# XuZhang1211/PVPUFormer

Hardware: AMD Instinct MI355X
Metric: 448x448 images/sec fwd+bwd, ViT-B VPUFormer (higher is better)
Workload: dtype bf16

## Files before the change

include/vpu_hip.h:

```cpp
#ifndef VPU_HIP_H
#define VPU_HIP_H
#include <stdint.h>

#ifdef __cplusplus
extern "C" {
#endif

#define VPU_BF16 0
#define VPU_F32 1

#define VPU_EPI_BIAS 1
#define VPU_EPI_PREACT 2
#define VPU_EPI_GELU 4
#define VPU_EPI_RELU 8
#define VPU_EPI_DGELU 16
#define VPU_EPI_DRELU 32
#define VPU_EPI_RESID 64
#define VPU_EPI_AFFINE 128
#define VPU_EPI_ACCUM 256
#define VPU_EPI_OUT_F32 512
#define VPU_EPI_SAVE_DGELU 1024
#define VPU_EPI_MULAUX 2048

typedef struct vpu_gemm_desc {
// ... 162 lines not shown
                             void* stream);
int vpu_pixel_shuffle2_gn_stats(const void* in, void* out, const float* bias, double* stats, int32_t B, int32_t h, int32_t w,
                                int32_t C, int32_t dtype, void* stream);
int vpu_groupnorm_apply(const void* x, const float* w, const float* b, void* y, float* mean, float* rstd, const double* stats,
                        int32_t B, int64_t HW, int32_t C, float eps, int32_t gelu, int32_t dtype, void* stream);
int vpu_pixel_unshuffle2_nblk(int32_t C);
int vpu_pixel_unshuffle2_sums(const void* in, void* out, float* part, int32_t B, int32_t h, int32_t w, int32_t C,
                              int32_t dtype, void* stream);
int vpu_groupnorm_nchunk(void);
int vpu_groupnorm_fwd(const void* x, const float* w, const float* b, void* y, float* mean, float* rstd, double* stats,
                      int32_t B, int64_t HW, int32_t C, float eps, int32_t gelu, int32_t dtype, void* stream);
int vpu_groupnorm_bwd(const void* dy, const void* x, const float* w, const float* b, const float* mean,
                      const float* rstd, void* dx, float* part, double* stats, int32_t B, int64_t HW, int32_t C,
                      int32_t gelu, int32_t dtype, void* stream);
int vpu_bilinear_cl_fwd(const void* in, int32_t ld_in, void* out, int32_t ld_out, int32_t B, int32_t h, int32_t w,
                        int32_t H, int32_t W, int32_t C, int32_t dtype, void* stream);
int vpu_bilinear_cl_bwd(const void* dout, int32_t ld_out, void* din, int32_t ld_in, int32_t B, int32_t h, int32_t w,
                        int32_t H, int32_t W, int32_t C, int32_t dtype, void* stream);
int vpu_upsum_relu(void* io, const void* const* z, const int32_t* h, const int32_t* w, int32_t n, int32_t B, int32_t H,
                   int32_t W, int32_t C, int32_t dtype, void* stream);
int vpu_head_grad_fused(const void* dfn, const void* y, const float* inv, const float* dout, const void* x, const float* w,
                        const float* mask, void* dx, float* part, float* part_b, int64_t rows, int64_t HW, int32_t C,
                        int32_t dtype, void* stream);
int vpu_gate_stats(const void* Q, const void* Kt, float* cg, int32_t* argq, float* sg, int32_t* argc, int32_t B,
                   int32_t nq, int32_t N, int32_t C, int32_t dtype, void* stream);
int vpu_gate_apply(const void* x, const float* cg, const float* sg, void* out, int32_t B, int32_t N, int32_t C,
                   int32_t dtype, void* stream);
int vpu_gate_bwd(const void* dout, const void* x, const float* cg, const int32_t* argq, const float* sg,
                 const int32_t* argc, void* dx, int32_t accum, void* dQ, void* dK, float* part, int32_t B, int32_t nq,
                 int32_t N, int32_t C, int32_t dtype, void* stream);
int vpu_gate_fwd_n(const void* const* Q, const void* const* K, const void* x, void* const* out, float* cg, int32_t* argq,
                   float* sg, int32_t* argc, int32_t n, int32_t B, int32_t nq, int32_t N, int32_t C, int32_t dtype, void* stream);
int vpu_gate_bwd_n(const void* const* dout, const void* x, const float* cg, const int32_t* argq, const float* sg,
                   const int32_t* argc, void* dx, int32_t accum, void* const* dQ, void* const* dK, float* part, int32_t n,
                   int32_t B, int32_t nq, int32_t N, int32_t C, int32_t dtype, void* stream);
int vpu_convseg_fwd(const void* x, const float* w, const float* bias, const float* mask, float* out, int64_t rows,
                    int64_t HW, int32_t C, int32_t dtype, void* stream);
int vpu_convseg_bwd_nblk(int64_t rows);
int vpu_convseg_bwd(const float* dout, const void* x, const float* w, const float* mask, void* dx, int32_t accum,
                    float* part, float* part_b, int64_t rows, int64_t HW, int32_t C, int32_t dtype, void* stream);

int vpu_upsample_ac_fwd(const float* in, float* out, int64_t planes, int32_t h, int32_t w, int32_t H, int32_t W,
                        void* stream);
int vpu_upsample_ac_bwd(const float* dout, float* din, int64_t planes, int32_t h, int32_t w, int32_t H, int32_t W,
                        void* stream);
int vpu_p2cl_fwd_bwd(const float* prob, const float* gt, const int32_t* slot_mask_idx, const float* override_masks,
// ... 28 lines not shown
```

pvpuformer_amd/_lib.py:

```python
import ctypes as C
import os

_HERE = os.path.dirname(os.path.abspath(__file__))
LIB_PATH = os.path.join(_HERE, os.environ.get("VPU_LIB_FILE") or
                        ("libvpu_hip_diag.so" if os.environ.get("VPU_LIB_DIAG", "0") == "1" else "libvpu_hip.so"))

BF16, F32 = 0, 1

EPI_BIAS, EPI_PREACT, EPI_GELU, EPI_RELU, EPI_DGELU, EPI_DRELU = 1, 2, 4, 8, 16, 32
EPI_RESID, EPI_AFFINE, EPI_ACCUM, EPI_OUT_F32 = 64, 128, 256, 512
EPI_SAVE_DGELU, EPI_MULAUX = 1024, 2048


class GemmDesc(C.Structure):
    _fields_ = [
        ("A", C.c_void_p), ("B", C.c_void_p), ("C", C.c_void_p), ("bias", C.c_void_p), ("resid", C.c_void_p),
        ("aux", C.c_void_p), ("preact", C.c_void_p),
        ("M", C.c_int32), ("N", C.c_int32), ("K", C.c_int32),
        ("lda", C.c_int32), ("ldb", C.c_int32), ("ldc", C.c_int32), ("ldr", C.c_int32), ("ldaux", C.c_int32),
        ("batch", C.c_int32), ("inner", C.c_int32),
        ("sAo", C.c_int64), ("sAi", C.c_int64), ("sBo", C.c_int64), ("sBi", C.c_int64),
        ("sCo", C.c_int64), ("sCi", C.c_int64), ("sRo", C.c_int64), ("sRi", C.c_int64),
        ("transA", C.c_int32), ("transB", C.c_int32), ("dtype", C.c_int32), ("flags", C.c_int32),
        ("resid_period", C.c_int32),
# ... 67 lines not shown
    "vpu_mask_bbox": [_P, _F, _P, _I, _P, _I, _I, _I, _P],
    "vpu_masked_argmax": [_P, _P, _P, _I, _I, _I, _P],
    "vpu_error_masks": [_P, _P, _P, _P, _I, _I, _P],
    "vpu_roi_resize_batched": [_P, _I, _P, _I, _I, _I, _I, _P],
    "vpu_roi_paste_batched": [_P, _I, _P, _I, _I, _F, _F, _I, _P],
    "vpu_click_keys_batched": [_P, _I, _P, _P, _P, _I, _I, _I, _P],
    "vpu_disk_maps": [_P, _P, _P, _I, _I, _I, _I, _F, _P],
    "vpu_patch_im2col": [_P, _P, _P, _I, _I, _I, _I, _I, _I, _P],
    "vpu_patch_im2col_prenorm": [_P, _P, _P, _I, _I, _I, _I, _I, _I, _P],
    "vpu_patch_im2col_floor": [_P, _P, _P, _I, _I, _I, _I, _I, _I, _I, _P],
    "vpu_window_permute": [_P, _P, _I, _I, _I, _I, _I, _I, _P],
    "vpu_space_to_depth2_crop": [_P, _P, _I, _I, _I, _I, _I, _P],
    "vpu_pixel_shuffle2": [_P, _P, _P, _I, _I, _I, _I, _I, _I, _P],
    "vpu_pixel_shuffle2_gn_stats": [_P, _P, _P, _P, _I, _I, _I, _I, _I, _P],
    "vpu_groupnorm_apply": [_P, _P, _P, _P, _P, _P, _P, _I, _L, _I, _F, _I, _I, _P],
    "vpu_pixel_unshuffle2_nblk": [_I],
    "vpu_pixel_unshuffle2_sums": [_P, _P, _P, _I, _I, _I, _I, _I, _P],
    "vpu_groupnorm_nchunk": [],
    "vpu_groupnorm_fwd": [_P, _P, _P, _P, _P, _P, _P, _I, _L, _I, _F, _I, _I, _P],
    "vpu_groupnorm_bwd": [_P, _P, _P, _P, _P, _P, _P, _P, _P, _I, _L, _I, _I, _I, _P],
    "vpu_bilinear_cl_fwd": [_P, _I, _P, _I, _I, _I, _I, _I, _I, _I, _I, _P],
    "vpu_bilinear_cl_bwd": [_P, _I, _P, _I, _I, _I, _I, _I, _I, _I, _I, _P],
    "vpu_head_grad_fused": [_P, _P, _P, _P, _P, _P, _P, _P, _P, _P, _L, _L, _I, _I, _P],
    "vpu_upsum_relu": [_P, C.POINTER(C.c_void_p), C.POINTER(C.c_int32), C.POINTER(C.c_int32), _I, _I, _I, _I, _I, _I, _P],
    "vpu_gate_stats": [_P, _P, _P, _P, _P, _P, _I, _I, _I, _I, _I, _P],
    "vpu_gate_apply": [_P, _P, _P, _P, _I, _I, _I, _I, _P],
    "vpu_gate_bwd": [_P, _P, _P, _P, _P, _P, _P, _I, _P, _P, _P, _I, _I, _I, _I, _I, _P],
    "vpu_gate_fwd_n": [C.POINTER(C.c_void_p), C.POINTER(C.c_void_p), _P, C.POINTER(C.c_void_p), _P, _P, _P, _P, _I, _I, _I, _I, _I, _I, _P],
    "vpu_gate_bwd_n": [C.POINTER(C.c_void_p), _P, _P, _P, _P, _P, _P, _I, C.POINTER(C.c_void_p), C.POINTER(C.c_void_p), _P, _I, _I, _I,
                       _I, _I, _I, _P],
    "vpu_convseg_fwd": [_P, _P, _P, _P, _P, _L, _L, _I, _I, _P],
    "vpu_convseg_bwd_nblk": [_L],
    "vpu_convseg_bwd": [_P, _P, _P, _P, _P, _I, _P, _P, _L, _L, _I, _I, _P],
    "vpu_upsample_ac_fwd": [_P, _P, _L, _I, _I, _I, _I, _P],
    "vpu_upsample_ac_bwd": [_P, _P, _L, _I, _I, _I, _I, _P],
    "vpu_p2cl_fwd_bwd": [_P, _P, _P, _P, _P, _P, _F, _I, _I, _I, _I, _P],
    "vpu_p2cl_up_nband": [_I, _I],
    "vpu_p2cl_up_fwd_bwd": [_P, _P, _P, _P, _P, _P, _F, _I, _I, _I, _I, _I, _I, _P],
    "vpu_nfl_dice_scratch_doubles": [_I],
    "vpu_nfl_dice_fwd_bwd": [_P, _P, _P, _P, _P, _F, _F, _I, _L, _P],
    "vpu_loss_finalize": [_P, _P, _I, _I, C.c_double, _F, _F, _F, _F, _P, _P],
    "vpu_adam_step": [_P, _P, _P, _P, _P, _L, _F, _F, _F, _F, _F, _I, _F, _P],
    "vpu_adam_step_groups": [_P, _P, _P, _P, _P, _L, _P, _P, _P, _I, _F, _F, _F, _I, _I, _F, _P],
    "vpu_adam_step_hyper": [_P, _P, _P, _P, _P, _L, _P, _P, _P, _P, _I, _F, _F, _F, _F, _I, _P],
    "vpu_gemm_set_option": [C.c_char_p, _I],
    "vpu_gemm_get_option": [C.c_char_p, C.POINTER(C.c_int32)],
# ... 40 lines not shown
```

pvpuformer_amd/csrc/spatial.hip:

```cpp
#include <stdlib.h>
#include "vpu_common.h"
#include "interp_ac.h"
#include "../../include/vpu_hip.h"

#define DISPATCH_T(dtype, ...)                                   \
    if ((dtype) == VPU_BF16) { using T = bf16_t; __VA_ARGS__ }   \
    else if ((dtype) == VPU_F32) { using T = float; __VA_ARGS__ } \
    else { vpu_set_error("bad dtype"); return VPU_ERR_ARG; }
#define ST reinterpret_cast<hipStream_t>(stream)

namespace {

__constant__ float c_mean[3] = {0.485f, 0.456f, 0.406f};
__constant__ float c_std[3] = {0.229f, 0.224f, 0.225f};

template <typename T, bool NORM = true, bool VEC = true>
__global__ __launch_bounds__(256) void patch_im2col_kernel(const float* __restrict__ img4,
                                                           const float* __restrict__ disks, T* __restrict__ cols,
                                                           int B, int H, int W, int P, int wg) {
    const int gw = W / P, gh = H / P;
    const int K3 = 3 * P * P, K3P = (K3 + 7) / 8 * 8;
    const int Tn = gw * gh, KK = 2 * K3P, chunks = KK / 8;
    const int64_t total = (int64_t)B * Tn * chunks;
    const int nwx = gw / wg;
// ... 711 lines not shown
            for (int u = 0; u < 2 * R; ++u) {
                const int X = Xs + u;
                if (X >= 0 && X < W) {
                    float g[8];
                    load8(rowp + (int64_t)X * ld_out, g);
                    const float ww = wy * wx[u];
#pragma unroll
                    for (int j = 0; j < 8; ++j) acc[j] += ww * g[j];
                }
            }
        }
    }
#pragma unroll
    for (int j = 0; j < 8; ++j) acc[j] += __shfl_xor(acc[j], 32, 64);
    if ((wave & 1) && lane < 32) {
#pragma unroll
        for (int j = 0; j < 8; ++j) red[wave >> 1][ck][j] = acc[j];
    }
    __syncthreads();
    if (!(wave & 1) && lane < 32 && live) {
#pragma unroll
        for (int j = 0; j < 8; ++j) acc[j] += red[wave >> 1][ck][j];
        store8(din + pix * ld_in + ck * 8, acc);
    }
}

template <typename T>
__global__ __launch_bounds__(256) void gate_colmax_kernel(const T* __restrict__ Q, float* __restrict__ cg,
                                                          int* __restrict__ argq, int B, int nq, int C) {
    const int64_t i = (int64_t)blockIdx.x * 256 + threadIdx.x;
    if (i >= (int64_t)B * C) return;
    const int c = (int)(i % C), b = (int)(i / C);
    float mx = -INFINITY;
    int am = 0;
#pragma unroll 8
    for (int q = 0; q < nq; ++q) {
        const float v = to_f32(Q[((int64_t)b * nq + q) * C + c]);
        if (v > mx) { mx = v; am = q; }
    }
    cg[i] = sigmoid_f(mx);
    argq[i] = am;
}
template <typename T>
__global__ __launch_bounds__(256) void gate_rowmax_kernel(const T* __restrict__ K, float* __restrict__ sg,
                                                          int* __restrict__ argc, int64_t rows, int C) {
    const int lane = threadIdx.x & 63;
// ... 539 lines not shown
            for (int j = 0; j < 8; ++j) {
                dwa[j] += d * xv[j] * mk[j];
                const float t = iv * (g[j] - yv[j] * sdot) + d * wv[j] * mk[j];
                o[j] = xv[j] > 0.f ? t : 0.f;
            }
            store8(dx + row * C + c8, o);
        }
    }
#pragma unroll
    for (int j = 0; j < 8; ++j)
        for (int o = lpr; o < 64; o <<= 1) dwa[j] += __shfl_xor(dwa[j], o, 64);
    dba = wave_sum(dba);
    if (sub == 0) {
#pragma unroll
        for (int j = 0; j < 8; ++j) red[wave][c8 + j] = dwa[j];
    }
    if (lane == 0) redb[wave] = dba;
    __syncthreads();
    for (int c = threadIdx.x; c < C; c += 256)
        part[(int64_t)blockIdx.x * C + c] = red[0][c] + red[1][c] + red[2][c] + red[3][c];
    if (threadIdx.x == 0) part_b[blockIdx.x] = redb[0] + redb[1] + redb[2] + redb[3];
}

__global__ __launch_bounds__(256) void upsample_ac_fwd_kernel(const float* __restrict__ in, float* __restrict__ out,
                                                              int64_t planes, int h, int w, int H, int W) {
    const float sh = ac_scale(h, H), sw = ac_scale(w, W);
    const int64_t total = planes * H * W;
    for (int64_t i = (int64_t)blockIdx.x * 256 + threadIdx.x; i < total; i += (int64_t)gridDim.x * 256) {
        const int X = (int)(i % W), Y = (int)((i / W) % H);
        const int64_t pl = i / ((int64_t)W * H);
        out[i] = ac_sample(in + pl * h * w, w, h, w, sh, sw, Y, X);
    }
}
__global__ __launch_bounds__(256) void upsample_ac_bwd_kernel(const float* __restrict__ dout, float* __restrict__ din,
                                                              int64_t planes, int h, int w, int H, int W) {
    const float sh = H > 1 ? (float)(h - 1) / (float)(H - 1) : 0.f;
    const float sw = W > 1 ? (float)(w - 1) / (float)(W - 1) : 0.f;
    const float fh = sh > 0.f ? 1.f / sh : 0.f, fw = sw > 0.f ? 1.f / sw : 0.f;
    const int64_t total = planes * h * w;
    const bool small = total < ((int64_t)1 << 31);
    for (int64_t i = (int64_t)blockIdx.x * 256 + threadIdx.x; i < total; i += (int64_t)gridDim.x * 256) {
        int x, y;
        int64_t pl;
        if (small) {
            const unsigned iu = (unsigned)i, q = iu / (unsigned)w;
            x = (int)(iu - q * (unsigned)w); y = (int)(q % (unsigned)h); pl = q / (unsigned)h;
// ... 221 lines not shown
    if ((R == 4 || R == 8) && R >= split_min && C == 256) {
        const unsigned g2 = (unsigned)(8 * ((((int64_t)B * h * w + 1) / 2 + 7) / 8));
        DISPATCH_T(dtype,
                   if (R == 4) bilinear_cl_bwd_int4_kernel<T, 4><<<g2, 256, 0, ST>>>((const T*)dout, ld_out, (T*)din, ld_in, B, h, w);
                   else bilinear_cl_bwd_int4_kernel<T, 8><<<g2, 256, 0, ST>>>((const T*)dout, ld_out, (T*)din, ld_in, B, h, w);)
        return vpu_check_launch("vpu_bilinear_cl_bwd");
    }
    if (R == 2 || R == 4 || R == 8) {
        const int64_t nb8 = 8 * (((total + 255) / 256 + 7) / 8);
        const unsigned gi = (unsigned)(nb8 < 16384 ? nb8 : 16384);
        DISPATCH_T(dtype,
                   if (R == 2) bilinear_cl_bwd_int_kernel<T, 2><<<gi, 256, 0, ST>>>(
                       (const T*)dout, ld_out, (T*)din, ld_in, B, h, w, C);
                   else if (R == 4) bilinear_cl_bwd_int_kernel<T, 4><<<gi, 256, 0, ST>>>(
                       (const T*)dout, ld_out, (T*)din, ld_in, B, h, w, C);
                   else bilinear_cl_bwd_int_kernel<T, 8><<<gi, 256, 0, ST>>>(
                       (const T*)dout, ld_out, (T*)din, ld_in, B, h, w, C);)
        return vpu_check_launch("vpu_bilinear_cl_bwd");
    }
    DISPATCH_T(dtype, bilinear_cl_bwd_kernel<T><<<vpu_grid_for(total, 256, 16384), 256, 0, ST>>>(
        (const T*)dout, ld_out, (T*)din, ld_in, B, h, w, H, W, C);)
    return vpu_check_launch("vpu_bilinear_cl_bwd");
}
extern "C" int vpu_gate_stats(const void* Q, const void* Kt, float* cg, int32_t* argq, float* sg, int32_t* argc,
                              int32_t B, int32_t nq, int32_t N, int32_t C, int32_t dtype, void* stream) {
    vpu_clear_stale_error();
    DISPATCH_T(dtype,
               gate_colmax_kernel<T><<<vpu_grid_for((int64_t)B * C, 256), 256, 0, ST>>>((const T*)Q, cg, argq, B, nq, C);
               gate_rowmax_kernel<T><<<(unsigned)(((int64_t)B * N + 3) / 4), 256, 0, ST>>>((const T*)Kt, sg, argc,
                                                                                          (int64_t)B * N, C);)
    return vpu_check_launch("vpu_gate_stats");
}
extern "C" int vpu_gate_apply(const void* x, const float* cg, const float* sg, void* out, int32_t B, int32_t N,
                              int32_t C, int32_t dtype, void* stream) {
    vpu_clear_stale_error();
    if (C % 8) { vpu_set_error("gate_apply: C % 8"); return VPU_ERR_ARG; }
    const int64_t total = (int64_t)B * N * (C / 8);
    DISPATCH_T(dtype, gate_apply_kernel<T><<<vpu_grid_for(total, 256, 16384), 256, 0, ST>>>((const T*)x, cg, sg, (T*)out,
                                                                                           B, N, C);)
    return vpu_check_launch("vpu_gate_apply");
}
extern "C" int vpu_gate_bwd(const void* dout, const void* x, const float* cg, const int32_t* argq, const float* sg,
                            const int32_t* argc, void* dx, int32_t accum, void* dQ, void* dK, float* part, int32_t B,
                            int32_t nq, int32_t N, int32_t C, int32_t dtype, void* stream) {
    vpu_clear_stale_error();
    if (C % 8 || C > 2048) { vpu_set_error("gate_bwd: C % 8, C <= 2048"); return VPU_ERR_ARG; }
// ... 84 lines not shown
        return vpu_check_launch("vpu_convseg_bwd");
    }
    DISPATCH_T(dtype, convseg_bwd_kernel<T><<<nblk, 256, 0, ST>>>(dout, (const T*)x, w, mask, (T*)dx, accum, part,
                                                                 part_b, rows, HW, C, nblk);)
    return vpu_check_launch("vpu_convseg_bwd");
}
extern "C" int vpu_head_grad_fused(const void* dfn, const void* y, const float* inv, const float* dout, const void* x,
                                   const float* w, const float* mask, void* dx, float* part, float* part_b, int64_t rows,
                                   int64_t HW, int32_t C, int32_t dtype, void* stream) {
    vpu_clear_stale_error();
    if (dtype != VPU_BF16 || !(C == 64 || C == 128 || C == 256 || C == 512) || !dfn || !y || !inv || !dout || !x || !w ||
        !dx || !part || !part_b || rows < 1 ||
        (reinterpret_cast<uintptr_t>(dfn) | reinterpret_cast<uintptr_t>(y) | reinterpret_cast<uintptr_t>(x) |
         reinterpret_cast<uintptr_t>(dx)) % 16 != 0 ||
        (reinterpret_cast<uintptr_t>(w) | reinterpret_cast<uintptr_t>(mask)) % 32 != 0) {
        vpu_set_error("head_grad_fused: bf16, C in {64,128,256,512}, 16-byte aligned maps, 32-byte aligned w / mask");
        return VPU_ERR_ARG;
    }
    const int nblk = vpu_convseg_bwd_nblk(rows);
    head_grad_fused_kernel<<<nblk, 256, 0, ST>>>((const bf16_t*)dfn, (const bf16_t*)y, inv, dout, (const bf16_t*)x, w, mask,
                                                 (bf16_t*)dx, part, part_b, rows, HW, C, nblk);
    return vpu_check_launch("vpu_head_grad_fused");
}
extern "C" int vpu_upsample_ac_fwd(const float* in, float* out, int64_t planes, int32_t h, int32_t w, int32_t H,
                                   int32_t W, void* stream) {
    vpu_clear_stale_error();
    upsample_ac_fwd_kernel<<<vpu_grid_for(planes * H * W, 256, 65536), 256, 0, ST>>>(in, out, planes, h, w, H, W);
    return vpu_check_launch("vpu_upsample_ac_fwd");
}
extern "C" int vpu_upsample_ac_bwd(const float* dout, float* din, int64_t planes, int32_t h, int32_t w, int32_t H,
                                   int32_t W, void* stream) {
    vpu_clear_stale_error();
    upsample_ac_bwd_kernel<<<vpu_grid_for(planes * h * w, 256, 65536), 256, 0, ST>>>(dout, din, planes, h, w, H, W);
    return vpu_check_launch("vpu_upsample_ac_bwd");
}
```

pvpuformer_amd/engine.py:

```python
import contextlib
import math
from collections import OrderedDict

import numpy as np
import torch

from . import ops
from ._lib import (BF16, F32, EPI_BIAS, EPI_PREACT, EPI_GELU, EPI_RELU, EPI_DGELU, EPI_DRELU, EPI_RESID, EPI_AFFINE,
                   EPI_ACCUM, EPI_OUT_F32, EPI_SAVE_DGELU, EPI_MULAUX)


class Tape:
    __slots__ = ("fns", "out_grads", "done", "sim_low", "lane")

    def __init__(self):
        self.fns = []
        self.out_grads = [None, None, None]
        self.done = False
        self.sim_low = None
        self.lane = None

    def append(self, fn):
        s = self.lane
        if s is not None:
# ... 89 lines not shown
        import os
        self.use_flash = True
        self.use_side = os.environ.get("VPU_WGRAD_STREAM", "0") == "1"
        self.side = None
        self.fuse_ln_pe = True
        self.group_wgrad = True
        self.ride_wgrad = True
        self.wgrad_fill = 0.8
        hid = self.D * c["mlp_ratio"]
        blk = sum(((n + 255) // 256) * ((k + 127) // 128) for n, k in ((3 * self.D, self.D), (self.D, self.D), (hid, self.D), (self.D, hid)))
        pk = os.environ.get("VPU_WGRAD_PACK", "")
        k3 = ops.gemm_get_option("k3")
        k4_default = (k3 & 8) != 0
        self.pack_wgrad = pk == "1" or (pk != "0" and (blk < 0.95 * 256 or k4_default))
        self.k3_wgrad = (k3 & 1) != 0
        self.k4_wgrad = (k3 & 8) != 0
        self.wgrad_round = 256 if (self.k4_wgrad or not self.k3_wgrad) else 512
        self.wgrad_tn = 256 if self.k4_wgrad else 128
        self.unify_wgrad = True
        self.lazy_zero = True
        self.r5_fused = True
        self.xattn_split = max(1, int(os.environ.get("VPU_XATTN_SPLIT", "1")))
        self.neck_lanes = int(os.environ.get("VPU_NECK_LANES", "0"))
        self._tok_stream = None
        self._in_lanes = False
        self.dist_colsum = True
        self._pack_seen, self._pack_total = {}, {}
        self._pending_reports, self._reporting = [], False
        self.group_tiles = 256
        self.split_wgrad = True
        self._wq = []
        self._csq = []
        self._gq = []
        self._gq_out = set()
        self._frozen = set()
        self._token_rows = 0
        self.grad_ready_hook = None
        self.report_lag = max(1, int(os.environ.get("VPU_DIST_REPORT_LAG", "2")))

    def bind(self, named_params):
        self.names = OrderedDict()
        off = 0
        for n, p in named_params.items():
            self.names[n] = (off, tuple(p.shape), p.numel())
            off = _rup(off + p.numel(), 8)
        self.total = off
# ... 978 lines not shown
        a = self.groupnorm(a, "neck.down_4.4", B, 16 * NT, c4 // 2, False)
        a = self.linear(a, "neck.down_4.5.weight", "neck.down_4.5.bias", B * 16 * NT, o[0], c4 // 2)
        d4 = self.groupnorm(a, "neck.down_4.6", B, 16 * NT, o[0], True)
        c8 = max(o[1], D // 2)
        a = self.conv_t2(maps[1], "neck.down_8.0", B, g, g, D, c8, gn_next=True)
        a = self.groupnorm(a, "neck.down_8.1", B, 4 * NT, c8, False)
        a = self.linear(a, "neck.down_8.2.weight", "neck.down_8.2.bias", B * 4 * NT, o[1], c8)
        d8 = self.groupnorm(a, "neck.down_8.3", B, 4 * NT, o[1], True)
        a = self.linear(maps[2], "neck.down_16.0.weight", "neck.down_16.0.bias", M, o[2], D)
        d16 = self.groupnorm(a, "neck.down_16.1", B, NT, o[2], True)
        c32 = max(o[3], D * 2)
        h32 = g // 2
        a = self.conv_s2(maps[3], "neck.down_32.0", B, h32, h32, D, c32, g=g)
        a = self.groupnorm(a, "neck.down_32.1", B, h32 * h32, c32, False)
        a = self.linear(a, "neck.down_32.2.weight", "neck.down_32.2.bias", B * h32 * h32, o[3], c32)
        d32 = self.groupnorm(a, "neck.down_32.3", B, h32 * h32, o[3], True)
        feats = [(d4, 4 * g), (d8, 2 * g), (d16, g), (d32, h32)]
        if taps is not None:
            for i, (f, s) in enumerate(feats):
                taps[f"fpn{i}"] = f.t
        Cc = self.C
        Hs = 4 * g
        HW4 = Hs * Hs
        wf, ldf = self.W("head.fusion_conv.conv.weight"), 4 * Cc
        gf = self.G("head.fusion_conv.conv.weight")
        ys, zs = [], []
        ymask = [[False] for _ in range(4)]
        for i in range(4):
            f, s = feats[i]
            ys.append(self.linear(f, f"head.convs.{i}.conv.weight", f"head.convs.{i}.conv.bias", B * s * s, Cc, o[i],
                                  act="relu", pre_masked=ymask[i]))
        fused = Var(self._new(B * HW4, Cc))
        ops.gemm(ys[0].t, wf, fused.t, B * HW4, Cc, Cc, Cc, ldf, Cc, self.dt, flags=EPI_BIAS,
                 bias=self.Pm("head.fusion_conv.conv.bias"))
        for i in (1, 2, 3):
            s = feats[i][1]
            z = self._new(B * s * s, Cc)
            ops.gemm(ys[i].t, (wf[0], wf[1] + i * Cc), z, B * s * s, Cc, Cc, Cc, ldf, Cc, self.dt)
            zs.append((z, s, s))
        ops.upsum_relu(fused.t, zs, B, Hs, Hs, Cc, self.dt)
        relu_done = [False]
        if training:
            def bwd_fusion():
                if fused.g is None:
                    return
                if relu_done[0]:
                    dt_ = fused.g
                else:
                    dt_ = self._new(B * HW4, Cc)
                    ops.act_bwd(fused.g, Cc, fused.t, Cc, dt_, Cc, B * HW4, Cc, 0, self.dt)
                self._wgrad(dt_, Cc, ys[0].t, Cc, gf, Cc, Cc, B * HW4, ldc=ldf, bias="head.fusion_conv.conv.bias")
                fuse_mask = self.dt == BF16
                mk = dict(flags=EPI_DRELU, ldaux=Cc) if fuse_mask else {}
                self._dgrad(dt_, Cc, wf, ldf, ys[0], B * HW4, Cc, Cc, **(dict(mk, aux=ys[0].t) if fuse_mask else {}))
                ymask[0][0] = fuse_mask
                for i in (1, 2, 3):
                    s = feats[i][1]
                    dz = self._new(B * s * s, Cc)
                    ops.bilinear_cl_bwd(dt_, Cc, dz, Cc, B, s, s, Hs, Hs, Cc, self.dt)
                    self._wgrad(dz, Cc, ys[i].t, Cc, (gf[0], gf[1] + i * Cc), Cc, Cc, B * s * s, ldc=ldf)
                    self._dgrad(dz, Cc, (wf[0], wf[1] + i * Cc), ldf, ys[i], B * s * s, Cc, Cc,
                                **(dict(mk, aux=ys[i].t) if fuse_mask else {}))
                    ymask[i][0] = fuse_mask
            self.tape.append(bwd_fusion)
        seg = self._new(B * HW4, dtype=torch.float32)
        ops.convseg_fwd(fused.t, self.Pm("head.conv_seg.weight"), self.Pm("head.conv_seg.bias"), drop_mask, seg,
                        B * HW4, HW4, Cc)
        dm = c["head_d_model"]
        query = self.mlp(q_out, "head.ffn_layer.lin1", "head.ffn_layer.lin2", B * nq, dm, 2 * dm, Cc, "relu")
        qn, fn = Var(torch.empty_like(query.t)), Var(torch.empty_like(fused.t))
        inv_q, inv_f = self._new(B * nq, dtype=torch.float32), self._new(B * HW4, dtype=torch.float32)
        ops.l2norm_fwd(query.t, qn.t, inv_q, B * nq, Cc)
        ops.l2norm_fwd(fused.t, fn.t, inv_f, B * HW4, Cc)
        sim = self._new(B, nq, HW4, dtype=torch.float32)
        ops.gemm(qn.t, fn.t, sim, nq, HW4, Cc, Cc, Cc, HW4, self.dt, flags=EPI_OUT_F32 | EPI_AFFINE, post_mul=0.5,
                 post_add=0.5, batch=B, inner=1, sA=(nq * Cc, 0), sB=(HW4 * Cc, 0), sC=(nq * HW4, 0))
        if taps is not None:
            taps["seg_lowres"] = seg.view(B, 1, Hs, Hs)
            taps["sim_lowres"] = sim.view(B, nq, Hs, Hs)
            taps["fused"] = fused.t
        inst = self._new(B, 1, H, W_, dtype=torch.float32)
        ops.upsample_ac_fwd(seg, inst, B, Hs, Hs, H, W_)
        aux = None
        self.sim_low = sim.view(B, nq, Hs, Hs)
        if materialize_aux:
            aux = self._new(B, nq, H, W_, dtype=torch.float32)
            ops.upsample_ac_fwd(sim, aux, B * nq, Hs, Hs, H, W_)
        tape.sim_low = self.sim_low
        if training:
            def bwd_head():
                d_inst, d_aux, d_sim_low = tape.out_grads
                if d_aux is not None or d_sim_low is not None:
                    if d_sim_low is not None:
                        dsim = d_sim_low.view(B, nq, HW4)
                    else:
                        dsim = self._new(B, nq, HW4, dtype=torch.float32)
                        ops.upsample_ac_bwd(d_aux, dsim, B * nq, Hs, Hs, H, W_)
                    if self.dt == BF16:
                        dsim_t = self._new(B, nq, HW4)
                        ops.cast2d(dsim, HW4, dsim_t, HW4, B * nq, HW4)
                    else:
                        dsim_t = dsim
                    qn.g, fn.g = torch.empty_like(qn.t), torch.empty_like(fn.t)
                    ops.gemm(dsim_t, fn.t, qn.g, nq, Cc, HW4, HW4, Cc, Cc, self.dt, transB=True, alpha=0.5, batch=B,
                             inner=1, sA=(nq * HW4, 0), sB=(HW4 * Cc, 0), sC=(nq * Cc, 0))
                    ops.gemm(dsim_t, qn.t, fn.g, HW4, Cc, nq, HW4, Cc, Cc, self.dt, transA=True, transB=True, alpha=0.5,
                             batch=B, inner=1, sA=(nq * HW4, 0), sB=(nq * Cc, 0), sC=(HW4 * Cc, 0))
                    query.g = torch.empty_like(query.t)
                    ops.l2norm_bwd(qn.g, qn.t, inv_q, query.g, B * nq, Cc)
                    one_pass = d_inst is not None and self.dt == BF16 and Cc in (64, 128, 256, 512)
                    if not one_pass:
                        fused.g = torch.empty_like(fused.t)
                        ops.l2norm_bwd(fn.g, fn.t, inv_f, fused.g, B * HW4, Cc)
                if d_inst is not None:
# ... 308 lines not shown
```

pvpuformer_amd/ops.py:

```python
import ctypes as C

import torch

from . import _lib
from ._lib import (BF16, F32, EPI_BIAS, EPI_PREACT, EPI_GELU, EPI_RELU, EPI_DGELU, EPI_DRELU, EPI_RESID, EPI_AFFINE,
                   EPI_ACCUM, EPI_OUT_F32, EPI_SAVE_DGELU, EPI_MULAUX, GemmDesc)

TORCH_DTYPE = {BF16: torch.bfloat16, F32: torch.float32}


def code_of(t):
    if isinstance(t, tuple):
        t = t[0]
    if t.dtype == torch.bfloat16:
        return BF16
    if t.dtype == torch.float32:
        return F32
    raise TypeError(f"unsupported dtype {t.dtype}")


_raw_stream = getattr(torch._C, "_cuda_getCurrentRawStream", None)
_cur_device = getattr(torch._C, "_cuda_getDevice", None)


# ... 477 lines not shown
def gate_bwd_n(douts, x, cg, argq, sg, argc, dx, accum, dQs, dKs, part, B, nq, N, Cdim):
    _lib.call("vpu_gate_bwd_n", _ptr_array(douts), ptr(x), ptr(cg), ptr(argq), ptr(sg), ptr(argc), ptr(dx), int(accum),
              _ptr_array(dQs), _ptr_array(dKs), ptr(part), len(douts), B, nq, N, Cdim, code_of(x), _stream())


def convseg_fwd(x, w, bias, mask, out, rows, HW, Cdim):
    _lib.call("vpu_convseg_fwd", ptr(x), ptr(w), ptr(bias), ptr(mask), ptr(out), rows, HW, Cdim, code_of(x), _stream())


def convseg_bwd_nblk(rows):
    return _lib.load().vpu_convseg_bwd_nblk(rows)


def convseg_bwd(dout, x, w, mask, dx, accum, part, part_b, rows, HW, Cdim):
    _lib.call("vpu_convseg_bwd", ptr(dout), ptr(x), ptr(w), ptr(mask), ptr(dx), int(accum), ptr(part), ptr(part_b),
              rows, HW, Cdim, code_of(x), _stream())


def head_grad_fused(dfn, y, inv, dout, x, w, mask, dx, part, part_b, rows, HW, Cdim):
    _lib.call("vpu_head_grad_fused", ptr(dfn), ptr(y), ptr(inv), ptr(dout), ptr(x), ptr(w), ptr(mask), ptr(dx), ptr(part),
              ptr(part_b), rows, HW, Cdim, code_of(x), _stream())


def upsample_ac_fwd(inp, out, planes, h, w, H, W):
    _lib.call("vpu_upsample_ac_fwd", ptr(inp), ptr(out), planes, h, w, H, W, _stream())


def upsample_ac_bwd(dout, din, planes, h, w, H, W):
    _lib.call("vpu_upsample_ac_bwd", ptr(dout), ptr(din), planes, h, w, H, W, _stream())


def p2cl_fwd_bwd(prob, gt, slot_idx, override, loss_part, dprob, grad_scale, B, S, H, W):
    _lib.call("vpu_p2cl_fwd_bwd", ptr(prob), ptr(gt), ptr(slot_idx), ptr(override), ptr(loss_part), ptr(dprob),
              grad_scale, B, S, H, W, _stream())


def p2cl_up_fwd_bwd(sim_low, gt, slot_idx, override, loss_part, dsim_low, grad_scale, B, S, h, w, H, W):
    nband = _lib.load().vpu_p2cl_up_nband(h, w)
    bands = torch.empty(B * S, nband, device=sim_low.device, dtype=torch.float32)
    _lib.call("vpu_p2cl_up_fwd_bwd", ptr(sim_low), ptr(gt), ptr(slot_idx), ptr(override), ptr(bands), ptr(dsim_low),
              grad_scale, B, S, h, w, H, W, _stream())
    if loss_part is None:
        return bands
    torch.sum(bands, dim=1, out=loss_part.view(B * S))
    return loss_part

# ... 27 lines not shown
```

Baseline: 1001.

## Fuse segmentation-head backward into one pass and batch three-level bilinear backward

Adds a one-pass head backward kernel. It computes the similarity-grad product with the queries via MFMA, the l2norm correction, the conv_seg gradient, the ReLU mask and the weight/bias partial sums in a single sweep over the fused map. This replaces several separate kernels and GEMMs, so the large feature map is read fewer times. It also adds a kernel that computes bilinear backward for the ratio-2, 4 and 8 levels from one shared LDS window of the upstream gradient, instead of three passes over it. The cost is more complex, shape-restricted kernels: bf16 only, fixed C values, nq <= 64. The product is computed twice per tile to save registers.

```diff
diff --git a/include/vpu_hip.h b/include/vpu_hip.h
--- a/include/vpu_hip.h
+++ b/include/vpu_hip.h
@@ -208,6 +208,12 @@
 int vpu_head_grad_fused(const void* dfn, const void* y, const float* inv, const float* dout, const void* x, const float* w,
                         const float* mask, void* dx, float* part, float* part_b, int64_t rows, int64_t HW, int32_t C,
                         int32_t dtype, void* stream);
+int vpu_head_bwd_onepass_nblk(int32_t B, int64_t HW);
+int vpu_head_bwd_onepass(const void* x, const float* dsim, const float* dseg, const float* inv, const void* qn, const float* w,
+                         const float* mask, void* dx, void* dsi, float* part, float* part_b, int32_t B, int64_t HW,
+                         int32_t nq, int32_t C, int32_t dtype, void* stream);
+int vpu_bilinear_cl_bwd3(const void* dout, void* const* dz, const int32_t* h, const int32_t* w, int32_t B, int32_t H,
+                         int32_t W, int32_t C, int32_t dtype, void* stream);
 int vpu_gate_stats(const void* Q, const void* Kt, float* cg, int32_t* argq, float* sg, int32_t* argc, int32_t B,
                    int32_t nq, int32_t N, int32_t C, int32_t dtype, void* stream);
 int vpu_gate_apply(const void* x, const float* cg, const float* sg, void* out, int32_t B, int32_t N, int32_t C,
diff --git a/pvpuformer_amd/_lib.py b/pvpuformer_amd/_lib.py
--- a/pvpuformer_amd/_lib.py
+++ b/pvpuformer_amd/_lib.py
@@ -113,6 +113,9 @@
     "vpu_bilinear_cl_fwd": [_P, _I, _P, _I, _I, _I, _I, _I, _I, _I, _I, _P],
     "vpu_bilinear_cl_bwd": [_P, _I, _P, _I, _I, _I, _I, _I, _I, _I, _I, _P],
     "vpu_head_grad_fused": [_P, _P, _P, _P, _P, _P, _P, _P, _P, _P, _L, _L, _I, _I, _P],
+    "vpu_head_bwd_onepass_nblk": [_I, _L],
+    "vpu_head_bwd_onepass": [_P, _P, _P, _P, _P, _P, _P, _P, _P, _P, _P, _I, _L, _I, _I, _I, _P],
+    "vpu_bilinear_cl_bwd3": [_P, C.POINTER(C.c_void_p), C.POINTER(C.c_int32), C.POINTER(C.c_int32), _I, _I, _I, _I, _I, _P],
     "vpu_upsum_relu": [_P, C.POINTER(C.c_void_p), C.POINTER(C.c_int32), C.POINTER(C.c_int32), _I, _I, _I, _I, _I, _I, _P],
     "vpu_gate_stats": [_P, _P, _P, _P, _P, _P, _I, _I, _I, _I, _I, _P],
     "vpu_gate_apply": [_P, _P, _P, _P, _I, _I, _I, _I, _P],
diff --git a/pvpuformer_amd/csrc/spatial.hip b/pvpuformer_amd/csrc/spatial.hip
--- a/pvpuformer_amd/csrc/spatial.hip
+++ b/pvpuformer_amd/csrc/spatial.hip
@@ -757,6 +757,101 @@
 #pragma unroll
         for (int j = 0; j < 8; ++j) acc[j] += red[wave >> 1][ck][j];
         store8(din + pix * ld_in + ck * 8, acc);
+    }
+}
+
+constexpr int BW3_CG = 64;
+template <int R>
+__device__ __forceinline__ void bwd3_gather(const bf16_t* __restrict__ win, int Ys0, int Xs0, int y, int x, int h, int w,
+                                            int v0, int nv, int ckl, float (&acc)[8]) {
+    const int H = R * h, W = R * w;
+    const float sh = (float)h / (float)H, sw = (float)w / (float)W;
+    const int Xs = R * x - R / 2, Ys = R * y - R / 2;
+    float wx[2 * R];
+#pragma unroll
+    for (int u = 0; u < 2 * R; ++u) {
+        const int X = Xs + u;
+        int x0, x1; float lx;
+        src_index_half(X < 0 ? 0 : X, sw, w, x0, x1, lx);
+        const float wgt = (x0 == x ? 1.f - lx : 0.f) + (x1 == x ? lx : 0.f);
+        wx[u] = (X >= 0 && X < W) ? wgt : 0.f;
+    }
+    for (int v = v0; v < v0 + nv; ++v) {
+        const int Y = Ys + v;
+        if (Y < 0 || Y >= H) continue;
+        int y0, y1; float ly;
+        src_index_half(Y, sh, h, y0, y1, ly);
+        const float wy = (y0 == y ? 1.f - ly : 0.f) + (y1 == y ? ly : 0.f);
+        const bf16_t* rowp = win + ((Y - Ys0) * 16 + (Xs - Xs0)) * BW3_CG + ckl * 8;
+#pragma unroll
+        for (int u = 0; u < 2 * R; ++u) {
+            const int X = Xs + u;
+            if (X >= 0 && X < W) {
+                float g[8];
+                load8(rowp + u * BW3_CG, g);
+                const float ww = wy * wx[u];
+#pragma unroll
+                for (int j = 0; j < 8; ++j) acc[j] += ww * g[j];
+            }
+        }
+    }
+}
+template <bool SPLIT8>
+__global__ __launch_bounds__(256) void bilinear_cl_bwd3_kernel(const bf16_t* __restrict__ dout, bf16_t* __restrict__ dz2,
+                                                               bf16_t* __restrict__ dz4, bf16_t* __restrict__ dz8, int B,
+                                                               int h8, int w8, int C) {
+    __shared__ __attribute__((aligned(16))) bf16_t win[16 * 16 * BW3_CG];
+    __shared__ float red[3][8][8];
+    const int H = 8 * h8, W = 8 * w8, ncg = C / BW3_CG;
+    const int64_t nblk = (int64_t)B * h8 * w8 * ncg, per = (nblk + 7) / 8;
+    const int64_t bb = ((int64_t)blockIdx.x & 7) * per + ((int64_t)blockIdx.x >> 3);
+    if (((int64_t)blockIdx.x >> 3) >= per || bb >= nblk) return;
+    const int c0 = (int)(bb % ncg) * BW3_CG;
+    const int64_t pix8 = bb / ncg;
+    const int x8 = (int)(pix8 % w8), y8 = (int)((pix8 / w8) % h8), b = (int)(pix8 / ((int64_t)w8 * h8));
+    const int Ys0 = 8 * y8 - 4, Xs0 = 8 * x8 - 4;
+    for (int i = threadIdx.x; i < 16 * 16 * (BW3_CG / 8); i += 256) {
+        const int ck = i & (BW3_CG / 8 - 1), px = i / (BW3_CG / 8);
+        const int Y = Ys0 + (px >> 4), X = Xs0 + (px & 15);
+        uint4 v = make_uint4(0, 0, 0, 0);
+        if (Y >= 0 && Y < H && X >= 0 && X < W)
+            v = *reinterpret_cast<const uint4*>(dout + (((int64_t)b * H + Y) * W + X) * C + c0 + ck * 8);
+        *reinterpret_cast<uint4*>(win + px * BW3_CG + ck * 8) = v;
+    }
+    __syncthreads();
+    const int lane = threadIdx.x & 63, wave = threadIdx.x >> 6;
+    const int ckl = lane & 7, sub = lane >> 3;
+    float acc[8] = {0.f, 0.f, 0.f, 0.f, 0.f, 0.f, 0.f, 0.f};
+    if (wave < 2) {
+        const int pp = wave * 8 + sub;
+        const int y = 4 * y8 + (pp >> 2), x = 4 * x8 + (pp & 3);
+        bwd3_gather<2>(win, Ys0, Xs0, y, x, 4 * h8, 4 * w8, 0, 4, ckl, acc);
+        store8(dz2 + (((int64_t)b * 4 * h8 + y) * (4 * w8) + x) * C + c0 + ckl * 8, acc);
+    } else if (wave == 2) {
+        if (sub < 4) {
+            const int y = 2 * y8 + (sub >> 1), x = 2 * x8 + (sub & 1);
+            bwd3_gather<4>(win, Ys0, Xs0, y, x, 2 * h8, 2 * w8, 0, 8, ckl, acc);
+            store8(dz4 + (((int64_t)b * 2 * h8 + y) * (2 * w8) + x) * C + c0 + ckl * 8, acc);
+        }
+    } else if (SPLIT8) {
+        if (sub < 4) {
+            bwd3_gather<8>(win, Ys0, Xs0, y8, x8, h8, w8, sub * 4, 4, ckl, acc);
+            if (sub > 0) {
+#pragma unroll
+                for (int j = 0; j < 8; ++j) red[sub - 1][ckl][j] = acc[j];
+            }
+        }
+    } else if (sub == 0) {
+        bwd3_gather<8>(win, Ys0, Xs0, y8, x8, h8, w8, 0, 16, ckl, acc);
+        store8(dz8 + pix8 * C + c0 + ckl * 8, acc);
+    }
+    if (SPLIT8) {
+        __syncthreads();
+        if (wave == 3 && sub == 0) {
+#pragma unroll
+            for (int j = 0; j < 8; ++j) acc[j] = (acc[j] + red[0][ckl][j]) + (red[1][ckl][j] + red[2][ckl][j]);
+            store8(dz8 + pix8 * C + c0 + ckl * 8, acc);
+        }
     }
 }
 
@@ -1342,6 +1437,139 @@
     if (threadIdx.x == 0) part_b[blockIdx.x] = redb[0] + redb[1] + redb[2] + redb[3];
 }
 
+constexpr int HB_QS = 72;
+constexpr int HB_TPB = 16;
+static inline size_t head_bwd_lds_bytes(int C) { return (size_t)C * HB_QS * 2 + (size_t)C * 6 * 4 + 16; }
+template <int C>
+__global__ __launch_bounds__(256, 2) void head_bwd_onepass_kernel(const bf16_t* __restrict__ x, const float* __restrict__ dsim,
+                                                               const float* __restrict__ dseg, const float* __restrict__ inv,
+                                                               const bf16_t* __restrict__ qn, const float* __restrict__ w,
+                                                               const float* __restrict__ mask, bf16_t* __restrict__ dx,
+                                                               bf16_t* __restrict__ dsi, float* __restrict__ part,
+                                                               float* __restrict__ part_b, int HW, int nq) {
+    extern __shared__ __attribute__((aligned(16))) char hb_smem[];
+    constexpr int NT = C / 16, NP = C / 32;
+    bf16_t* qT = reinterpret_cast<bf16_t*>(hb_smem);
+    float* wl = reinterpret_cast<float*>(hb_smem + (size_t)C * HB_QS * 2);
+    float* ml = wl + C;
+    float* red = ml + C;
+    float* redb = red + 4 * C;
+    const int b = blockIdx.y;
+    const int lane = threadIdx.x & 63, wave = threadIdx.x >> 6;
+    const int g = lane >> 4, pl = lane & 15;
+    for (int i = threadIdx.x; i < C * HB_QS / 8; i += 256) reinterpret_cast<uint4*>(qT)[i] = make_uint4(0, 0, 0, 0);
+    for (int c = threadIdx.x; c < C; c += 256) {
+        wl[c] = w[c];
+        ml[c] = mask ? mask[(int64_t)b * C + c] : 1.f;
+    }
+    __syncthreads();
+    for (int i = threadIdx.x; i < nq * (C / 8); i += 256) {
+        const int q = i / (C / 8), c8 = (i % (C / 8)) * 8;
+        const bf16x8_t v = *reinterpret_cast<const bf16x8_t*>(qn + ((int64_t)b * nq + q) * C + c8);
+#pragma unroll
+        for (int j = 0; j < 8; ++j) qT[(c8 + j) * HB_QS + q] = v[j];
+    }
+    __syncthreads();
+    float dwa[NP][8];
+#pragma unroll
+    for (int k = 0; k < NP; ++k)
+#pragma unroll
+        for (int j = 0; j < 8; ++j) dwa[k][j] = 0.f;
+    float dba = 0.f;
+    const int ntile = (HW + 15) >> 4;
+    const int t0 = blockIdx.x * HB_TPB, t1 = t0 + HB_TPB < ntile ? t0 + HB_TPB : ntile;
+    for (int t = t0 + wave; t < t1; t += 4) {
+        const int p = t * 16 + pl;
+        const bool live = p < HW;
+        const int64_t row = (int64_t)b * HW + p;
+        bf16x8_t xr[NP];
+#pragma unroll
+        for (int k = 0; k < NP; ++k) {
+            uint4 v = make_uint4(0, 0, 0, 0);
+            if (live) v = *reinterpret_cast<const uint4*>(x + row * C + k * 32 + g * 8);
+            xr[k] = __builtin_bit_cast(bf16x8_t, v);
+        }
+        const float iv = live ? inv[row] : 0.f, d = live ? dseg[row] : 0.f;
+        bf16x8_t bfr[2];
+#pragma unroll
+        for (int s = 0; s < 2; ++s)
+#pragma unroll
+            for (int i = 0; i < 8; ++i) {
+                const int q = s * 32 + g * 8 + i;
+                const bool on = live && q < nq;
+                const int64_t at = ((int64_t)b * nq + q) * HW + p;
+                const float v = on ? dsim[at] : 0.f;
+                bfr[s][i] = (bf16_t)v;
+                if (on) dsi[at] = (bf16_t)(v * iv);
+            }
+        constexpr int NH = NT / 2, KH = NP / 2;
+        f32x4_t acc[NH];
+        auto product = [&](int h) {
+#pragma unroll
+            for (int u = 0; u < NH; ++u) {
+                const int tt = h * NH + u;
+                acc[u] = f32x4_t{0.f, 0.f, 0.f, 0.f};
+                const int ch = (tt >> 1) * 32 + (pl >> 2) * 8 + (tt & 1) * 4 + (pl & 3);
+#pragma unroll
+                for (int s = 0; s < 2; ++s) {
+                    if (s * 32 >= nq) continue;
+                    const uint4 av = *reinterpret_cast<const uint4*>(qT + ch * HB_QS + s * 32 + g * 8);
+                    acc[u] = __builtin_amdgcn_mfma_f32_16x16x32_bf16(__builtin_bit_cast(bf16x8_t, av), bfr[s], acc[u], 0, 0, 0);
+                }
+            }
+        };
+        float sdot = 0.f;
+#pragma unroll
+        for (int h = 0; h < 2; ++h) {
+            product(h);
+#pragma unroll
+            for (int kk = 0; kk < KH; ++kk)
+#pragma unroll
+                for (int j = 0; j < 8; ++j) sdot += 0.5f * acc[2 * kk + (j >> 2)][j & 3] * ((float)xr[h * KH + kk][j] * iv);
+        }
+        sdot += __shfl_xor(sdot, 16, 64);
+        sdot += __shfl_xor(sdot, 32, 64);
+        if (g == 0) dba += d;
+#pragma unroll
+        for (int h = 0; h < 2; ++h) {
+            product(h);
+#pragma unroll
+            for (int kk = 0; kk < KH; ++kk) {
+                const int k = h * KH + kk;
+                float wv[8], mk[8], o[8];
+                load8(wl + k * 32 + g * 8, wv);
+                load8(ml + k * 32 + g * 8, mk);
+#pragma unroll
+                for (int j = 0; j < 8; ++j) {
+                    const float xf = (float)xr[k][j], gj = 0.5f * acc[2 * kk + (j >> 2)][j & 3];
+                    dwa[k][j] += d * xf;
+                    const float tv = iv * (gj - xf * iv * sdot) + d * wv[j] * mk[j];
+                    o[j] = xf > 0.f ? tv : 0.f;
+                }
+                if (live) store8(dx + row * C + k * 32 + g * 8, o);
+            }
+        }
+    }
+#pragma unroll
+    for (int k = 0; k < NP; ++k)
+#pragma unroll
+        for (int j = 0; j < 8; ++j) {
+            float v = dwa[k][j];
+            v += __shfl_xor(v, 1, 64);
+            v += __shfl_xor(v, 2, 64);
+            v += __shfl_xor(v, 4, 64);
+            v += __shfl_xor(v, 8, 64);
+            if (pl == 0) red[wave * C + k * 32 + g * 8 + j] = v;
+        }
+    dba = wave_sum(dba);
+    if (lane == 0) redb[wave] = dba;
+    __syncthreads();
+    const int64_t pr = (int64_t)b * gridDim.x + blockIdx.x;
+    for (int c = threadIdx.x; c < C; c += 256)
+        part[pr * C + c] = (red[c] + red[C + c] + red[2 * C + c] + red[3 * C + c]) * ml[c];
+    if (threadIdx.x == 0) part_b[pr] = redb[0] + redb[1] + redb[2] + redb[3];
+}
+
 __global__ __launch_bounds__(256) void upsample_ac_fwd_kernel(const float* __restrict__ in, float* __restrict__ out,
                                                               int64_t planes, int h, int w, int H, int W) {
     const float sh = ac_scale(h, H), sw = ac_scale(w, W);
@@ -1609,6 +1837,27 @@
         (const T*)dout, ld_out, (T*)din, ld_in, B, h, w, H, W, C);)
     return vpu_check_launch("vpu_bilinear_cl_bwd");
 }
+extern "C" int vpu_bilinear_cl_bwd3(const void* dout, void* const* dz, const int32_t* h, const int32_t* w, int32_t B,
+                                    int32_t H, int32_t W, int32_t C, int32_t dtype, void* stream) {
+    vpu_clear_stale_error();
+    bool ok = dtype == VPU_BF16 && dout && dz && h && w && B >= 1 && H >= 8 && W >= 8 && C >= BW3_CG && C % BW3_CG == 0 &&
+              reinterpret_cast<uintptr_t>(dout) % 16 == 0;
+    for (int i = 0; ok && i < 3; ++i)
+        ok = dz[i] && reinterpret_cast<uintptr_t>(dz[i]) % 16 == 0 && h[i] * (2 << i) == H && w[i] * (2 << i) == W;
+    if (!ok) {
+        vpu_set_error("bilinear_cl_bwd3: bf16, C % 64 == 0, three 16-byte aligned levels of ratio 2, 4 and 8 (in this order)");
+        return VPU_ERR_ARG;
+    }
+    const int64_t nblk = (int64_t)B * h[2] * w[2] * (C / BW3_CG);
+    const unsigned grid = (unsigned)(8 * ((nblk + 7) / 8));
+    if (C == 256)
+        bilinear_cl_bwd3_kernel<true><<<grid, 256, 0, ST>>>((const bf16_t*)dout, (bf16_t*)dz[0], (bf16_t*)dz[1], (bf16_t*)dz[2], B,
+                                                            h[2], w[2], C);
+    else
+        bilinear_cl_bwd3_kernel<false><<<grid, 256, 0, ST>>>((const bf16_t*)dout, (bf16_t*)dz[0], (bf16_t*)dz[1], (bf16_t*)dz[2], B,
+                                                             h[2], w[2], C);
+    return vpu_check_launch("vpu_bilinear_cl_bwd3");
+}
 extern "C" int vpu_gate_stats(const void* Q, const void* Kt, float* cg, int32_t* argq, float* sg, int32_t* argc,
                               int32_t B, int32_t nq, int32_t N, int32_t C, int32_t dtype, void* stream) {
     vpu_clear_stale_error();
@@ -1739,6 +1988,35 @@
                                                  (bf16_t*)dx, part, part_b, rows, HW, C, nblk);
     return vpu_check_launch("vpu_head_grad_fused");
 }
+extern "C" int vpu_head_bwd_onepass_nblk(int32_t B, int64_t HW) {
+    vpu_clear_stale_error();
+    const int64_t ntile = (HW + 15) / 16;
+    return (int)(B * ((ntile + HB_TPB - 1) / HB_TPB));
+}
+extern "C" int vpu_head_bwd_onepass(const void* x, const float* dsim, const float* dseg, const float* inv, const void* qn,
+                                    const float* w, const float* mask, void* dx, void* dsi, float* part, float* part_b,
+                                    int32_t B, int64_t HW, int32_t nq, int32_t C, int32_t dtype, void* stream) {
+    vpu_clear_stale_error();
+    if (dtype != VPU_BF16 || !(C == 64 || C == 128 || C == 256 || C == 512) || !x || !dsim || !dseg || !inv || !qn || !w ||
+        !dx || !dsi || !part || !part_b || B < 1 || B > 65535 || HW < 1 || HW > (1 << 30) || nq < 1 || nq > 64 ||
+        (reinterpret_cast<uintptr_t>(x) | reinterpret_cast<uintptr_t>(dx) | reinterpret_cast<uintptr_t>(qn)) % 16 != 0) {
+        vpu_set_error("head_bwd_onepass: bf16, C in {64,128,256,512}, 1 <= nq <= 64, 16-byte aligned maps and queries");
+        return VPU_ERR_ARG;
+    }
+    const int nbi = vpu_head_bwd_onepass_nblk(1, HW);
+    const dim3 grid(nbi, B);
+    const size_t lds = head_bwd_lds_bytes(C);
+#define VPU_HEAD_BWD(C_)                                                                                                  \
+    {                                                                                                                     \
+        static VpuDevOnce once;                                                                                           \
+        if (auto todo = once.pending()) { VPU_SET_LDS((int)head_bwd_lds_bytes(C_), head_bwd_onepass_kernel<C_>); }        \
+        head_bwd_onepass_kernel<C_><<<grid, 256, lds, ST>>>((const bf16_t*)x, dsim, dseg, inv, (const bf16_t*)qn, w, mask, \
+                                                            (bf16_t*)dx, (bf16_t*)dsi, part, part_b, (int)HW, nq);        \
+    }
+    if (C == 64) VPU_HEAD_BWD(64) else if (C == 128) VPU_HEAD_BWD(128) else if (C == 256) VPU_HEAD_BWD(256) else VPU_HEAD_BWD(512)
+#undef VPU_HEAD_BWD
+    return vpu_check_launch("vpu_head_bwd_onepass");
+}
 extern "C" int vpu_upsample_ac_fwd(const float* in, float* out, int64_t planes, int32_t h, int32_t w, int32_t H,
                                    int32_t W, void* stream) {
     vpu_clear_stale_error();
diff --git a/pvpuformer_amd/engine.py b/pvpuformer_amd/engine.py
--- a/pvpuformer_amd/engine.py
+++ b/pvpuformer_amd/engine.py
@@ -135,6 +135,7 @@
         self.r5_fused = True
         self.xattn_split = max(1, int(os.environ.get("VPU_XATTN_SPLIT", "1")))
         self.neck_lanes = int(os.environ.get("VPU_NECK_LANES", "0"))
+        self.head_onepass = int(os.environ.get("VPU_HEAD_ONEPASS", "1") or 1)
         self._tok_stream = None
         self._in_lanes = False
         self.dist_colsum = True
@@ -1159,6 +1160,8 @@
         Cc = self.C
         Hs = 4 * g
         HW4 = Hs * Hs
+        head_new = (self.head_onepass and self.dt == BF16 and Cc in (64, 128, 256, 512) and nq <= 64 and
+                    [f[1] * r for f, r in zip(feats[1:], (2, 4, 8))] == [Hs] * 3)
         wf, ldf = self.W("head.fusion_conv.conv.weight"), 4 * Cc
         gf = self.G("head.fusion_conv.conv.weight")
         ys, zs = [], []
@@ -1191,10 +1194,17 @@
                 mk = dict(flags=EPI_DRELU, ldaux=Cc) if fuse_mask else {}
                 self._dgrad(dt_, Cc, wf, ldf, ys[0], B * HW4, Cc, Cc, **(dict(mk, aux=ys[0].t) if fuse_mask else {}))
                 ymask[0][0] = fuse_mask
+                if head_new:
+                    dzs = [self._new(B * feats[i][1] ** 2, Cc) for i in (1, 2, 3)]
+                    ops.bilinear_cl_bwd3(dt_, [(dzs[i - 1], feats[i][1], feats[i][1]) for i in (1, 2, 3)], B, Hs, Hs, Cc,
+                                         self.dt)
                 for i in (1, 2, 3):
                     s = feats[i][1]
-                    dz = self._new(B * s * s, Cc)
-                    ops.bilinear_cl_bwd(dt_, Cc, dz, Cc, B, s, s, Hs, Hs, Cc, self.dt)
+                    if head_new:
+                        dz = dzs[i - 1]
+                    else:
+                        dz = self._new(B * s * s, Cc)
+                        ops.bilinear_cl_bwd(dt_, Cc, dz, Cc, B, s, s, Hs, Hs, Cc, self.dt)
                     self._wgrad(dz, Cc, ys[i].t, Cc, (gf[0], gf[1] + i * Cc), Cc, Cc, B * s * s, ldc=ldf)
                     self._dgrad(dz, Cc, (wf[0], wf[1] + i * Cc), ldf, ys[i], B * s * s, Cc, Cc,
                                 **(dict(mk, aux=ys[i].t) if fuse_mask else {}))
@@ -1227,6 +1237,28 @@
         if training:
             def bwd_head():
                 d_inst, d_aux, d_sim_low = tape.out_grads
+                if head_new and int(self.head_onepass) == 1 and d_inst is not None and (d_aux is not None or d_sim_low is not None):
+                    if d_sim_low is not None:
+                        dsim = d_sim_low.view(B, nq, HW4)
+                    else:
+                        dsim = self._new(B, nq, HW4, dtype=torch.float32)
+                        ops.upsample_ac_bwd(d_aux, dsim, B * nq, Hs, Hs, H, W_)
+                    dseg = self._new(B * HW4, dtype=torch.float32)
+                    ops.upsample_ac_bwd(d_inst, dseg, B, Hs, Hs, H, W_)
+                    nb = ops.head_bwd_onepass_nblk(B, HW4)
+                    part, part_b = self._new(nb, Cc, dtype=torch.float32), self._new(nb, dtype=torch.float32)
+                    dsi = self._new(B, nq, HW4)
+                    fused.g = torch.empty_like(fused.t)
+                    ops.head_bwd_onepass(fused.t, dsim, dseg, inv_f, qn.t, self.Pm("head.conv_seg.weight"), drop_mask, fused.g,
+                                         dsi, part, part_b, B, HW4, nq, Cc)
+                    relu_done[0] = True
+                    qn.g = torch.empty_like(qn.t)
+                    ops.gemm(dsi, fused.t, qn.g, nq, Cc, HW4, HW4, Cc, Cc, self.dt, transB=True, alpha=0.5, batch=B,
+                             inner=1, sA=(nq * HW4, 0), sB=(HW4 * Cc, 0), sC=(nq * Cc, 0))
+                    query.g = torch.empty_like(query.t)
+                    ops.l2norm_bwd(qn.g, qn.t, inv_q, query.g, B * nq, Cc)
+                    self._convseg_sums(part, part_b, nb, Cc)
+                    return
                 if d_aux is not None or d_sim_low is not None:
                     if d_sim_low is not None:
                         dsim = d_sim_low.view(B, nq, HW4)
diff --git a/pvpuformer_amd/ops.py b/pvpuformer_amd/ops.py
--- a/pvpuformer_amd/ops.py
+++ b/pvpuformer_amd/ops.py
@@ -523,6 +523,21 @@
               ptr(part_b), rows, HW, Cdim, code_of(x), _stream())
 
 
+def head_bwd_onepass_nblk(B, HW):
+    return _lib.load().vpu_head_bwd_onepass_nblk(B, HW)
+
+
+def head_bwd_onepass(x, dsim, dseg, inv, qn, w, mask, dx, dsi, part, part_b, B, HW, nq, Cdim):
+    _lib.call("vpu_head_bwd_onepass", ptr(x), ptr(dsim), ptr(dseg), ptr(inv), ptr(qn), ptr(w), ptr(mask), ptr(dx), ptr(dsi),
+              ptr(part), ptr(part_b), B, HW, nq, Cdim, code_of(x), _stream())
+
+
+def bilinear_cl_bwd3(dout, dzs, B, H, W, Cdim, dtype):
+    hs = (C.c_int32 * 3)(*[m[1] for m in dzs])
+    ws = (C.c_int32 * 3)(*[m[2] for m in dzs])
+    _lib.call("vpu_bilinear_cl_bwd3", ptr(dout), _ptr_array([m[0] for m in dzs]), hs, ws, B, H, W, Cdim, dtype, _stream())
+
+
 def upsample_ac_fwd(inp, out, planes, h, w, H, W):
     _lib.call("vpu_upsample_ac_fwd", ptr(inp), ptr(out), planes, h, w, H, W, _stream())
 
```

After: 1000. About the same (-0.1%).
